# qinjr/SCoRe

Measured on AMD Instinct MI355X. Metric: train samples/sec @ batch=1024, higher is better.
Workload: dtype f32

## Files before the change

### score_amd/csrc/embed.hip

```cpp
#include <string.h>
#include "common.h"
#include "kernels.h"

__global__ void gather_rows_kernel(const float* __restrict__ table, int D4, const int32_t* __restrict__ idx,
                                   int64_t n_chunks, float* __restrict__ out) {
  int64_t i = (int64_t)blockIdx.x * blockDim.x + threadIdx.x;
  int64_t stride = (int64_t)gridDim.x * blockDim.x;
  for (; i < n_chunks; i += stride) {
    int64_t r = i / D4;
    int c = (int)(i - r * D4);
    int64_t row = idx[r];
    st4(out + i * 4, ld4(table + (row * D4 + c) * 4));
  }
}

extern "C" int score_gather_fwd(const float* table, int64_t n_rows, int32_t D, const int32_t* idx,
                                int64_t n_idx, float* out, void* stream) {
  if (!table || !idx || !out || n_rows <= 0 || n_idx < 0) return SCORE_E_BADARG;
  if (D <= 0 || (D & 3)) return SCORE_E_SHAPE;
  if (n_idx == 0) return 0;
  int64_t n_chunks = n_idx * (D / 4);
  int blocks = (int)(cdiv64(n_chunks, 256) < 4096 ? cdiv64(n_chunks, 256) : 4096);
  hipLaunchKernelGGL(gather_rows_kernel, dim3(blocks), dim3(256), 0, (hipStream_t)stream, table, D / 4, idx,
                     n_chunks, out);
// ... 138 lines not shown
#pragma unroll
  for (int k = 0; k < KMAX; ++k) {
    r[k] = 0.f;
    if (k < K) {
      r[k] = fmaxf(red[k] + c, 0.f);
      rmax = fmaxf(rmax, r[k]);
      rsum += r[k];
    }
  }
  float p[KMAX];
  float den = 0.f;
#pragma unroll
  for (int k = 0; k < KMAX; ++k) {
    p[k] = (k < K) ? expf(r[k] - rmax) : 0.f;
    den += p[k];
  }
  const float inv_den = 1.0f / den;
#pragma unroll
  for (int j = 0; j < SPL; ++j) {
    if (!ok[j]) continue;
    float4 o = make_float4(0.f, 0.f, 0.f, 0.f);
#pragma unroll
    for (int k = 0; k < KMAX; ++k)
      if (k < K) o = fma4(p[k] * inv_den, v1[j][k], o);
    st4(cc.out1 + (int64_t)u * cc.ld1 + (gl + j * GS) * 4, o);
    const float fk = (float)K;
    st4(cc.out2 + (int64_t)u * cc.ld2 + (gl + j * GS) * 4,
        make_float4(sum2[j].x / fk, sum2[j].y / fk, sum2[j].z / fk, sum2[j].w / fk));
  }
  if (unit_ok) {
    for (int i = gl; i < 2 * K; i += GS) {
      float val = rsum;
      float rv = 0.f;
#pragma unroll
      for (int k = 0; k < KMAX; ++k)
        if (i == k) rv = r[k];
      if (i < K) {
        val = (float)K * rv;
        cc.rsave[(int64_t)u * K + i] = rv;
      }
      cc.info[(int64_t)u * cc.ldi + i] = val;
    }
  }
}

__device__ __forceinline__ void atomic_add4(float* d, float4 v) {
  atomicAdd(d, v.x); atomicAdd(d + 1, v.y); atomicAdd(d + 2, v.z); atomicAdd(d + 3, v.w);
}

__device__ __forceinline__ void rows_in_flight(float4& row, const float4& last) {
  asm volatile("" : "+v"(row.x), "+v"(row.y), "+v"(row.z), "+v"(row.w) : "v"(last.w));
}

template <int KMAX, int SPL, bool ATOMIC>
__global__ __launch_bounds__(256, (KMAX <= 10 && SPL == 1) ? 4 : 1) void coattn_bwd_kernel_t(const CoattnArgs a) {
  extern __shared__ float lds[];
  const int ci = (int)blockIdx.x >= a.c[1].first_block ? 1 : 0;
  const CoattnCall& cc = a.c[ci];
  const int GS = cc.GS, nslots = cc.nslots, F = cc.F, K = a.K, D4 = a.D4, n_units = a.n_units;
  const int mode = a.mode;
  const bool all_rows = a.all_rows != 0;
  const int lane = threadIdx.x & 63;
  const int wib = threadIdx.x >> 6;
  const int upw = 64 / GS;
  const int gl = lane & (GS - 1);
  const int grp = lane / GS;
  const int Dx = nslots * 4;
  const int D = D4 * 4;
  const int my_blocks = (ci == 0 ? min(a.c[1].first_block, (int)gridDim.x) : (int)gridDim.x) - cc.first_block;
  const int waves_total = my_blocks * 4;
  const int blk = (int)blockIdx.x - cc.first_block;
  const int wave0 = blk * 4 + wib;
  const float* __restrict__ table = a.table;
  float* __restrict__ gtable = a.gtable;
  const float* __restrict__ W = cc.W;

  bool sok[SPL];
  int f[SPL], coff[SPL];
  float4 w1[SPL], w2[SPL], dw1[SPL], dw2[SPL];
#pragma unroll
  for (int j = 0; j < SPL; ++j) {
    int s = gl + j * GS;
    sok[j] = s < nslots;
    int sc = sok[j] ? s : 0;
    f[j] = sc / D4;
    coff[j] = (sc - f[j] * D4) * 4;
    w1[j] = w2[j] = dw1[j] = dw2[j] = make_float4(0.f, 0.f, 0.f, 0.f);
    if (mode == 0) {
      w1[j] = ld4(W + Dx + sc * 4);
      w2[j] = ld4(W + 2 * Dx + sc * 4);
    }
  }

  const int n_iter = (n_units + waves_total * upw - 1) / (waves_total * upw);
  for (int it = 0; it < n_iter; ++it) {
    const int unit = (it * waves_total + wave0) * upw + grp;
    const bool unit_ok = unit < n_units;
    const int u = unit_ok ? unit : 0;
    const int ub = u / a.T;
    const int64_t ui = (int64_t)ub * a.Tidx + (u - ub * a.T);
    const int32_t* __restrict__ i1 = cc.idx1 + ui * K * F;
    const int32_t* __restrict__ i2 = cc.idx2 + ui * K * F;
    float4 g1[SPL], g2[SPL];
    bool ok[SPL];
#pragma unroll
    for (int j = 0; j < SPL; ++j) {
      ok[j] = unit_ok && sok[j];
      g1[j] = g2[j] = make_float4(0.f, 0.f, 0.f, 0.f);
      if (ok[j]) {
        g1[j] = ld4(cc.g1 + (int64_t)u * cc.ld1 + (gl + j * GS) * 4);
        g2[j] = ld4(cc.g2 + (int64_t)u * cc.ld2 + (gl + j * GS) * 4);
      }
    }
    if (mode == 1) {
#pragma unroll
      for (int k = 0; k < KMAX; ++k) {
#pragma unroll
        for (int j = 0; j < SPL; ++j) {
          if (!ok[j] || k >= K) continue;
          if (!ATOMIC) continue;
          int64_t r1 = i1[k * F + f[j]], r2 = i2[k * F + f[j]];
          r1 = (uint64_t)r1 < a.n_rows ? r1 : 0;
          r2 = (uint64_t)r2 < a.n_rows ? r2 : 0;
          if (r1 != 0) atomic_add4(gtable + r1 * D + coff[j], g1[j]);
          if (r2 != 0) atomic_add4(gtable + r2 * D + coff[j], g2[j]);
        }
      }
      continue;
    }

    int32_t r1[SPL][KMAX], rb2[SPL][KMAX];
    float dp[KMAX];
#pragma unroll
    for (int k = 0; k < KMAX; ++k) {
      const int kc = k < K ? k : K - 1;
#pragma unroll
      for (int j = 0; j < SPL; ++j) {
        r1[j][k] = i1[kc * F + f[j]];
        rb2[j][k] = i2[kc * F + f[j]];
      }
    }
    __builtin_amdgcn_sched_barrier(0);
#pragma unroll
    for (int k = 0; k < KMAX; ++k) {
      dp[k] = 0.f;
#pragma unroll
      for (int j = 0; j < SPL; ++j) {
        r1[j][k] = (uint32_t)r1[j][k] < a.n_rows ? r1[j][k] : 0;
        rb2[j][k] = (uint32_t)rb2[j][k] < a.n_rows ? rb2[j][k] : 0;
      }
    }
#pragma unroll
    for (int j = 0; j < SPL; ++j) {
      float4 v1[KMAX];
#pragma unroll
      for (int k = 0; k < KMAX; ++k) v1[k] = ld4(table + (int64_t)r1[j][k] * D + coff[j]);
#pragma unroll
      for (int k = 0; k < KMAX; ++k) rows_in_flight(v1[k], v1[KMAX - 1]);
#pragma unroll
      for (int k = 0; k < KMAX; ++k) {
        const bool live = ok[j] && k < K;
        v1[k].x = live ? v1[k].x : 0.f; v1[k].y = live ? v1[k].y : 0.f;
        v1[k].z = live ? v1[k].z : 0.f; v1[k].w = live ? v1[k].w : 0.f;
        r1[j][k] = live ? r1[j][k] : 0;
        rb2[j][k] = live ? rb2[j][k] : 0;
        dp[k] += dot4(v1[k], g1[j]);
      }
    }
    float r[KMAX], p[KMAX], gik[KMAX];
    float rmax = 0.f, gsum = 0.f;
#pragma unroll
    for (int k = 0; k < KMAX; ++k) {
      const int kc = k < K ? k : K - 1;
      const float rv = cc.rsave[(int64_t)u * K + kc];
      const float g2v = cc.ginfo[(int64_t)u * cc.ldi + K + kc];
      gik[k] = cc.ginfo[(int64_t)u * cc.ldi + kc];
      r[k] = (k < K) ? rv : 0.f;
      rmax = fmaxf(rmax, r[k]);
      gsum += (k < K) ? g2v : 0.f;
    }
    float den = 0.f;
#pragma unroll
    for (int k = 0; k < KMAX; ++k) {
      p[k] = (k < K) ? expf(r[k] - rmax) : 0.f;
      den += p[k];
    }
    const float inv_den = 1.0f / den;
    float pdp = 0.f;
    group_sum_n<KMAX>(dp, GS);
#pragma unroll
    for (int k = 0; k < KMAX; ++k) {
      p[k] *= inv_den;
      dp[k] = (k < K) ? dp[k] : 0.f;
      pdp += p[k] * dp[k];
    }
    float dz[KMAX];
    float dzs = 0.f;
#pragma unroll
    for (int k = 0; k < KMAX; ++k) {
      dz[k] = 0.f;
      if (k < K) {
        float dr = (float)K * gik[k] + gsum + p[k] * (dp[k] - pdp);
        dz[k] = r[k] > 0.f ? dr : 0.f;
        dzs += dz[k];
      }
    }
    if (unit_ok && gl == 0) cc.dzsum[u] = dzs;
    if (!ATOMIC && unit_ok) {
      for (int i = gl; i < K; i += GS) {
        float pv = 0.f, dv = 0.f;
#pragma unroll
        for (int k = 0; k < KMAX; ++k)
          if (i == k) { pv = p[k]; dv = dz[k]; }
        cc.pcoef[(int64_t)u * K + i] = pv;
        cc.dzcoef[(int64_t)u * K + i] = dv;
      }
    }
    const float invK = 1.0f / (float)K;
    bool act[KMAX];
#pragma unroll
    for (int k = 0; k < KMAX; ++k) act[k] = all_rows || (k < K && r[k] > 0.f);
#pragma unroll
    for (int j = 0; j < SPL; ++j) {
      float4 xr[KMAX];
#pragma unroll
      for (int k = 0; k < KMAX; ++k) {
        const int32_t lr = act[k] ? r1[j][k] : 0;
        xr[k] = ld4(table + (int64_t)lr * D + coff[j]);
      }
#pragma unroll
      for (int k = 0; k < KMAX; ++k) {
        dw1[j] = fma4(dz[k], xr[k], dw1[j]);
        if (ATOMIC && r1[j][k] != 0) {
          float4 d1 = fma4(dz[k], w1[j],
                           make_float4(p[k] * g1[j].x, p[k] * g1[j].y, p[k] * g1[j].z, p[k] * g1[j].w));
          atomic_add4(gtable + (int64_t)r1[j][k] * D + coff[j], d1);
        }
      }
    }
#pragma unroll
    for (int j = 0; j < SPL; ++j) {
      const float4 g2k = make_float4(g2[j].x * invK, g2[j].y * invK, g2[j].z * invK, g2[j].w * invK);
      float4 y[KMAX];
#pragma unroll
      for (int k = 0; k < KMAX; ++k) {
        const int32_t lr = act[k] ? rb2[j][k] : 0;
        y[k] = ld4(table + (int64_t)lr * D + coff[j]);
      }
#pragma unroll
      for (int k = 0; k < KMAX; ++k) {
        dw2[j] = fma4(dz[k], y[k], dw2[j]);
        if (ATOMIC && rb2[j][k] != 0) atomic_add4(gtable + (int64_t)rb2[j][k] * D + coff[j], fma4(dz[k], w2[j], g2k));
      }
    }
  }
  if (mode == 1) return;
  float* mine = lds + ((wib * upw + grp) * 2) * Dx;
#pragma unroll
  for (int j = 0; j < SPL; ++j) {
    if (!sok[j]) continue;
    st4(mine + (gl + j * GS) * 4, dw1[j]);
    st4(mine + Dx + (gl + j * GS) * 4, dw2[j]);
  }
  __syncthreads();
  const int nsrc = 4 * upw;
  for (int e = threadIdx.x; e < 2 * Dx; e += blockDim.x) {
    float s = 0.f;
    for (int q = 0; q < nsrc; ++q) s += lds[q * 2 * Dx + e];
    cc.slab[(int64_t)blk * 2 * Dx + e] = s;
  }
}

#define COATTN_DISPATCH(KERNEL, EXTRA, SPLV, KV, ...)                                     \
  do {                                                                                    \
    if (SPLV == 1) {                                                                      \
      if (KV <= 4) { hipLaunchKernelGGL((KERNEL<4, 1 EXTRA>), __VA_ARGS__); }             \
      else if (KV <= 10) { hipLaunchKernelGGL((KERNEL<10, 1 EXTRA>), __VA_ARGS__); }      \
      else if (KV <= 20) { hipLaunchKernelGGL((KERNEL<20, 1 EXTRA>), __VA_ARGS__); }      \
      else { hipLaunchKernelGGL((KERNEL<32, 1 EXTRA>), __VA_ARGS__); }                    \
    } else if (SPLV == 2) {                                                               \
      if (KV <= 4) { hipLaunchKernelGGL((KERNEL<4, 2 EXTRA>), __VA_ARGS__); }             \
      else if (KV <= 10) { hipLaunchKernelGGL((KERNEL<10, 2 EXTRA>), __VA_ARGS__); }      \
      else if (KV <= 20) { hipLaunchKernelGGL((KERNEL<20, 2 EXTRA>), __VA_ARGS__); }      \
      else { hipLaunchKernelGGL((KERNEL<32, 2 EXTRA>), __VA_ARGS__); }                    \
    } else {                                                                              \
      if (KV <= 10) { hipLaunchKernelGGL((KERNEL<10, 4 EXTRA>), __VA_ARGS__); }           \
      else { hipLaunchKernelGGL((KERNEL<20, 4 EXTRA>), __VA_ARGS__); }                    \
    }                                                                                     \
  } while (0)
#define COMMA_TRUE , true
#define COMMA_FALSE , false

static int coattn_check(const void* table, int64_t n_rows, int D, int F, int K, int B, int T) {
  if (!table || n_rows <= 0 || B <= 0 || T <= 0) return SCORE_E_BADARG;
  if (D <= 0 || (D & 3) || D > 256 || F <= 0 || K <= 0 || K > 32) return SCORE_E_SHAPE;
  if (F * (D / 4) > 256) return SCORE_E_SHAPE;
  if (F * (D / 4) > 128 && K > 20) return SCORE_E_SHAPE;
  return 0;
}

int score_coattn_fwd_multi(CoattnArgs& a, int ncalls, int D, int B, hipStream_t s) {
  int spl = 1, total = 0;
  a.D4 = D / 4;
  a.n_units = B * a.T;
  if (a.Tidx <= 0) a.Tidx = a.T;
  if (a.n_rows == 0) a.n_rows = 0x80000000u;
  for (int c = 0; c < 2; ++c) {
    if (c >= ncalls) { a.c[c] = a.c[0]; a.c[c].first_block = 0x7fffffff; continue; }
    int SPLc;
    coattn_geom(D, a.c[c].F, &a.c[c].GS, &SPLc, &a.c[c].nslots);
    if (SPLc > spl) spl = SPLc;
    a.c[c].first_block = total;
    total += (int)cdiv64(cdiv64(a.n_units, 64 / a.c[c].GS), 4);
  }
  if (spl == 3) spl = 4;
  COATTN_DISPATCH(coattn_fwd_kernel, , spl, a.K, dim3(total), dim3(256), 0, s, a);
  SCORE_CHECK_LAUNCH();
  return 0;
}

int score_coattn_bwd_multi(CoattnArgs& a, int ncalls, int D, int B, float* const dW[2], float* scratch,
                           int64_t scratch_floats, int atomic_scatter, ColsumJobs* cq, hipStream_t s) {
  int spl = 1, total = 0, nblk[2] = {0, 0};
  size_t lds_bytes = 0;
  int64_t used = 0;
  a.D4 = D / 4;
  a.n_units = B * a.T;
  if (a.Tidx <= 0) a.Tidx = a.T;
  if (a.n_rows == 0) a.n_rows = 0x80000000u;
  for (int c = 0; c < 2; ++c) {
    if (c >= ncalls) { a.c[c] = a.c[0]; a.c[c].first_block = 0x7fffffff; continue; }
    int SPLc;
    coattn_geom(D, a.c[c].F, &a.c[c].GS, &SPLc, &a.c[c].nslots);
    if (SPLc > spl) spl = SPLc;
    int upw = 64 / a.c[c].GS, Dx = a.c[c].nslots * 4;
    int blocks = (int)cdiv64(cdiv64(a.n_units, upw), 4);
    if (blocks > 512) blocks = 512;
    nblk[c] = blocks;
    a.c[c].first_block = total;
    total += blocks;
    a.c[c].slab = scratch + used;
    used += (int64_t)blocks * 2 * Dx;
    size_t l = (size_t)4 * upw * 2 * Dx * sizeof(float);
    if (l > lds_bytes) lds_bytes = l;
  }
  if (a.mode == 0 && used > scratch_floats) return SCORE_E_WORKSPACE;
  if (spl == 3) spl = 4;
  if (atomic_scatter) COATTN_DISPATCH(coattn_bwd_kernel_t, COMMA_TRUE, spl, a.K, dim3(total), dim3(256), lds_bytes, s, a);
  else COATTN_DISPATCH(coattn_bwd_kernel_t, COMMA_FALSE, spl, a.K, dim3(total), dim3(256), lds_bytes, s, a);
  SCORE_CHECK_LAUNCH();
  if (a.mode == 0) {
    for (int c = 0; c < ncalls; ++c) {
      int Dx = a.c[c].nslots * 4;
      if (cq) SCORE_TRY(colsum_queue_add(cq, a.c[c].slab, nblk[c], 2 * Dx, 2 * Dx, dW[c] + Dx, 1));
      else SCORE_TRY(score_launch_colsum(a.c[c].slab, nblk[c], 2 * Dx, 2 * Dx, dW[c] + Dx, 1, scratch + used,
                                         scratch_floats - used, s));
    }
  }
  return 0;
}

extern "C" int score_coattn_fwd(const float* table, int64_t n_rows, int32_t D, int32_t F, int32_t K,
                                int32_t B, int32_t T, const int32_t* idx1, const int32_t* idx2,
                                const float* tgt, const float* W, const float* bias, float* out1,
                                int32_t ld1, float* out2, int32_t ld2, float* info, int32_t ldi,
                                float* rsave, int32_t mode, void* stream) {
  SCORE_TRY(coattn_check(table, n_rows, D, F, K, B, T));
  if (!idx1 || !idx2 || !out1 || !out2) return SCORE_E_BADARG;
  if (mode == 0 && (!tgt || !W || !bias || !info || !rsave)) return SCORE_E_BADARG;
  if ((ld1 & 3) || (ld2 & 3)) return SCORE_E_SHAPE;
  CoattnArgs a;
  memset(&a, 0, sizeof(a));
  a.table = table; a.K = K; a.T = T; a.mode = mode; a.n_rows = (uint32_t)(n_rows < 0x80000000ll ? n_rows : 0x80000000ll);
  CoattnCall& c = a.c[0];
  c.idx1 = idx1; c.idx2 = idx2; c.tgt = tgt; c.ldt = F * D; c.W = W; c.bias = bias;
  c.out1 = out1; c.ld1 = ld1; c.out2 = out2; c.ld2 = ld2; c.info = info; c.ldi = ldi; c.rsave = rsave; c.F = F;
  return score_coattn_fwd_multi(a, 1, D, B, (hipStream_t)stream);
}

extern "C" int score_coattn_bwd(const float* table, float* grad_table, int64_t n_rows, int32_t D, int32_t F,
                                int32_t K, int32_t B, int32_t T, const int32_t* idx1, const int32_t* idx2,
                                const float* W, const float* rsave, const float* g1, int32_t ld1,
                                const float* g2, int32_t ld2, const float* ginfo, int32_t ldi, float* dzsum,
                                float* dW, float* scratch, int64_t scratch_floats, int32_t mode, void* stream) {
  SCORE_TRY(coattn_check(table, n_rows, D, F, K, B, T));
  if (!grad_table || !idx1 || !idx2 || !g1 || !g2) return SCORE_E_BADARG;
  if (mode == 0 && (!W || !rsave || !ginfo || !dzsum || !dW || !scratch)) return SCORE_E_BADARG;
  if ((ld1 & 3) || (ld2 & 3)) return SCORE_E_SHAPE;
  CoattnArgs a;
  memset(&a, 0, sizeof(a));
  a.table = table; a.gtable = grad_table; a.K = K; a.T = T; a.mode = mode;
  a.n_rows = (uint32_t)(n_rows < 0x80000000ll ? n_rows : 0x80000000ll);
  CoattnCall& c = a.c[0];
  c.idx1 = idx1; c.idx2 = idx2; c.W = W; c.rsave = const_cast<float*>(rsave); c.g1 = g1; c.ld1 = ld1; c.g2 = g2; c.ld2 = ld2;
  c.ginfo = ginfo; c.ldi = ldi; c.dzsum = dzsum; c.F = F;
  float* dWs[2] = {dW, nullptr};
  return score_coattn_bwd_multi(a, 1, D, B, dWs, scratch, scratch_floats, 1, nullptr, (hipStream_t)stream);
}

__global__ void target_fwd_kernel(const float* __restrict__ table, int D4, int Fu, int Fi, int B,
                                  const int32_t* __restrict__ tu, const int32_t* __restrict__ ti,
                                  float* __restrict__ query, int ldq, float* __restrict__ head, int ldh,
// ... 126 lines not shown
```

### score_amd/csrc/engine.hip

```cpp
#include <string.h>
#include <stdlib.h>
#include <stdio.h>
#include <math.h>
#include <mutex>
#include <new>
#include "common.h"
#include "kernels.h"
#include "persample.h"

namespace {

const int FC1 = 200, FC2 = 80, AT1 = 80, AT2 = 40;
const int CASER_L = SCORE_CASER_L, CASER_HPAD = SCORE_CASER_HPAD;
const int MAX_ENTRIES = 48;

enum Family { FAM_SLICE, FAM_GCMC, FAM_G4R, FAM_CASER, FAM_DELF, FAM_DEEMS, FAM_SVDPP, FAM_SASREC };

struct Dims {
  int64_t N;
  int D, H, T, K, Fu, Fi, mt;
  int Du, Di, I, Dq, NI, Dk, Dhead, nstate;
  int Is[2];
  bool coattn, attn;
  Family family;
// ... 468 lines not shown
  HIPTRY(hipEventRecord((hipEvent_t)event, (hipStream_t)stream));
  return 0;
}
extern "C" int score_stream_wait_event(void* stream, void* event) {
  if (!event) return SCORE_E_BADARG;
  HIPTRY(hipStreamWaitEvent((hipStream_t)stream, (hipEvent_t)event, 0));
  return 0;
}
extern "C" int score_event_query(void* event) {
  if (!event) return SCORE_E_BADARG;
  const hipError_t e = hipEventQuery((hipEvent_t)event);
  return e == hipSuccess ? 0 : e == hipErrorNotReady ? 1 : (int)e;
}
extern "C" int score_event_synchronize(void* event) {
  if (!event) return SCORE_E_BADARG;
  HIPTRY(hipEventSynchronize((hipEvent_t)event));
  return 0;
}
static int side_stream_create(SideStream* sd) {
  int dev = 0;
  if (hipGetDevice(&dev) != hipSuccess) return SCORE_E_BADARG;
  hipStream_t st; hipEvent_t a, b, c;
  hipError_t e = hipStreamCreateWithFlags(&st, hipStreamNonBlocking);
  if (e != hipSuccess) return (int)e;
  if ((e = hipEventCreateWithFlags(&a, SCORE_DEVICE_EVENT_FLAGS)) != hipSuccess) { hipStreamDestroy(st); return (int)e; }
  if ((e = hipEventCreateWithFlags(&b, SCORE_DEVICE_EVENT_FLAGS)) != hipSuccess) { hipEventDestroy(a); hipStreamDestroy(st); return (int)e; }
  if ((e = hipEventCreateWithFlags(&c, SCORE_DEVICE_EVENT_FLAGS)) != hipSuccess) { hipEventDestroy(a); hipEventDestroy(b); hipStreamDestroy(st); return (int)e; }
  sd->st = st; sd->fork = a; sd->join = b; sd->wx = c; sd->device = dev; sd->fwd_on = nullptr;
  return 0;
}
static void side_stream_release(SideStream* sd) {
  if (!sd->st) return;
  hipStreamSynchronize(sd->st);
  hipEventDestroy(sd->fork); hipEventDestroy(sd->join); hipEventDestroy(sd->wx);
  hipStreamDestroy(sd->st);
  sd->st = nullptr;
}
#define SCORE_MAX_DEVICES 16
static SideStream g_default_ctx[SCORE_MAX_DEVICES];
static std::mutex g_default_mu;
static int side_stream(const score_state_t* st, SideStream** out) {
  if (st && st->context) { *out = reinterpret_cast<SideStream*>(st->context); return 0; }
  int dev = 0;
  if (hipGetDevice(&dev) != hipSuccess || dev < 0 || dev >= SCORE_MAX_DEVICES) return SCORE_E_BADARG;
  std::lock_guard<std::mutex> lock(g_default_mu);
  SideStream& sd = g_default_ctx[dev];
  if (!sd.st) SCORE_TRY(side_stream_create(&sd));
  *out = &sd;
  return 0;
}
enum {
  DF_GRU_STEPWISE = 1, DF_HEAD_FUSED_ANY_B = 2, DF_GRU_F32_REC = 4, DF_NO_PANEL = 8, DF_PANEL_DX = 16, DF_SORT_LIB = 32,
  DF_HEAD_UNFUSED = 64, DF_ATTN_UNFUSED = 128, DF_SORT_OWN = 256, DF_NO_PS = 512, DF_PS_FWD_ONLY = 1024, DF_PS_BWD_ONLY = 2048,
  DF_ONE_STREAM = 4096, DF_G4R_COMPOSED = 8192, DF_PRODUCTS_LATE = 16384, DF_COATTN_ALL_ROWS = 32768
};
struct Flags {
  bool gru_stepwise, head_fused_any_b, gru_f32_rec, no_panel, panel_dx, sort_lib, head_unfused, attn_unfused, sort_own, no_ps,
      ps_fwd_only, ps_bwd_only, one_stream, g4r_composed, products_late, coattn_all_rows;
};
static inline Flags flags_of(const score_state_t* st) {
  auto on = [st](int bit) { return (st->debug_flags & bit) != 0; };
  Flags o;
  o.gru_stepwise = on(DF_GRU_STEPWISE); o.head_fused_any_b = on(DF_HEAD_FUSED_ANY_B); o.gru_f32_rec = on(DF_GRU_F32_REC);
  o.no_panel = on(DF_NO_PANEL); o.panel_dx = on(DF_PANEL_DX); o.sort_lib = on(DF_SORT_LIB); o.sort_own = on(DF_SORT_OWN);
  o.head_unfused = on(DF_HEAD_UNFUSED); o.attn_unfused = on(DF_ATTN_UNFUSED); o.no_ps = on(DF_NO_PS);
  o.ps_fwd_only = on(DF_PS_FWD_ONLY); o.ps_bwd_only = on(DF_PS_BWD_ONLY); o.one_stream = on(DF_ONE_STREAM);
  o.g4r_composed = on(DF_G4R_COMPOSED); o.products_late = on(DF_PRODUCTS_LATE); o.coattn_all_rows = on(DF_COATTN_ALL_ROWS);
  return o;
}
static int side_stream(const score_state_t* st, hipStream_t s, SideStream** out) {
  SideStream* real = nullptr;
  SCORE_TRY(side_stream(st, &real));
  if (!st || !flags_of(st).one_stream) { *out = real; return 0; }
  static thread_local SideStream inl;
  const hipStream_t was = inl.fwd_on;
  inl = *real; inl.st = s; inl.fwd_on = was;
  *out = &inl;
  return 0;
}
static inline int fork_side(SideStream* side, hipStream_t s) {
  HIPTRY(hipEventRecord(side->fork, s));
  HIPTRY(hipStreamWaitEvent(side->st, side->fork, 0));
  return 0;
}

#define G(call) SCORE_TRY(call)
static inline int gemm_mode_call(int x3, int tr, int M, int N, int K, const float* A, int lda, const float* B,
                                 int ldb, float* C, int ldc, const float* bias, int flags, float keep,
                                 const uint8_t* mask, uint64_t seed, float* scratch, int64_t scratch_floats,
                                 void* s) {
  return score_gemm(tr, M, N, K, A, lda, B, ldb, C, ldc, bias, flags | x3, keep, mask, seed, scratch, scratch_floats,
                    s);
}
#define EV(i) \
  do { if (stage_events && stage_events[i]) HIPTRY(hipEventRecord((hipEvent_t)stage_events[i], s)); } while (0)

static inline uint32_t clamp_rows(int64_t n) { return (uint32_t)(n < 0x80000000ll ? n : 0x80000000ll); }
static inline int global_batch(const score_state_t* st, int B) { return st->global_batch > 0 ? st->global_batch : B; }

struct Pass {
  Dims d; Params P; WS w; Flags fl;
  const score_state_t* st; const score_batch_t* bt;
  int B, T, BT, H;
  int x3, Bg;
  uint32_t n_rows;
  int64_t weff_stride;
  float rs;
  float* ws; const float* W; float* scratch;
  hipStream_t s;
};
static int pass_fill(Pass* c, const score_state_t* st, const score_batch_t* bt, void* stream) {
  const Dims& d = c->d;
  build_layout(d, nullptr, 0, &c->P);
  c->st = st; c->bt = bt; c->fl = flags_of(st);
  c->B = bt->B; c->T = active_T(d, bt); c->H = d.H; c->BT = c->B * c->T;
  build_ws(d, c->B, &c->w);
  if (c->w.total * 4 > st->workspace_bytes) return SCORE_E_WORKSPACE;
  c->x3 = st->gemm_mode == 1 ? GF_X3 : 0; c->Bg = global_batch(st, c->B); c->n_rows = clamp_rows(st->n_table_rows);
  c->weff_stride = weff_copy_stride(d); c->rs = (float)(1.0 / sqrt(1.0 + 1e-3));
  c->ws = st->workspace; c->W = st->w; c->scratch = c->ws + c->w.scratch;
// ... 1292 lines not shown
    HIPTRY(hipMemsetAsync(ws + w.dxside[sd], 0, (int64_t)BT * d.I * sizeof(float), s));
    const int Dx = d.Is[sd];
    float* dz = ws + w.gcmc_dz[sd];
    float* da = ws + w.gcmc_da[sd];
    G(gemm_mode_call(x3, 1, BT, Dx, 3 * H, ws + w.dxproj[sd], 3 * H, wxcat(c, sd), 3 * H, dz, Dx, nullptr, GF_RELUGRAD, 1.f,
                     reinterpret_cast<const uint8_t*>(ws + w.gcmc_z[sd]), 0, c.scratch, SF, s));
    G(gemm_queue_add(&gq, Dx, Dx, BT, ws + w.gcmc_a[sd], Dx, dz, Dx, gw + P.gm_c[sd], Dx));
    G(gemm_mode_call(x3, 1, BT, Dx, Dx, dz, Dx, W + P.gm_c[sd], Dx, da, Dx, nullptr, GF_RELUGRAD, 1.f,
                     reinterpret_cast<const uint8_t*>(ws + w.gcmc_a[sd]), 0, c.scratch, SF, s));
    G(gemm_queue_add(&gq, Dx, Dx, BT, ws + w.xside[sd], d.I, da, Dx, gw + P.gm_a[sd], Dx));
    G(gemm_mode_call(x3, 1, BT, Dx, Dx, da, Dx, W + P.gm_a[sd], Dx, ws + w.dxside[sd], d.I, nullptr, 0, 1.f, nullptr, 0,
                     c.scratch, SF, s));
  }
  return 0;
}

int bwd_dx_g4r(const Pass& c, BwdState* b) {
  const Dims& d = c.d; const WS& w = c.w; float* ws = c.ws; const int H = c.H, BT = c.BT; hipStream_t s = c.s;
  G(queue_gru_side(c, &b->q, b->gw, 0, b->gru_bias_rows));
  HIPTRY(hipMemsetAsync(ws + w.dxside[0], 0, (int64_t)BT * d.I * sizeof(float), s));
  G(gemm_mode_call(c.x3, 1, BT, d.Di, 3 * H, ws + w.dxproj[0], 3 * H, wxcat(c, 0), 3 * H, ws + w.dxside[0], d.I, nullptr, 0, 1.f,
                   nullptr, 0, c.scratch, w.scratch_floats, s));
  G(queue_gru_side(c, &b->q, b->gw, 1, b->gru_bias_rows));
  HIPTRY(hipMemsetAsync(ws + w.dxside[1], 0, (int64_t)BT * d.I * sizeof(float), s));
  return 0;
}

int bwd_close(const Pass& c, BwdState* b) {
  const Dims& d = c.d; const Params& P = c.P; const WS& w = c.w; const score_state_t* st = c.st; const score_batch_t* bt = c.bt;
  float* ws = c.ws; const float* W = c.W; float* gw = b->gw; float* grad_table = b->grad_table;
  const int B = c.B, x3 = c.x3; hipStream_t s = c.s;
  void* const* stage_events = b->stage_events;
  SideStream* side = b->side;
  GemmQueue& gq = b->q.gq;
  ColsumJobs& cq = b->q.cq;
  const int64_t half = slab_half(w);
  ReduceGroup rg; rg.n = rg.blocks = 0;
  const bool products_early = st->scatter_mode != 2 && !c.fl.products_late && gq.n > 0;
  const bool fin_side = st->grads_done_event != nullptr;
  const bool fin_early = products_early && fin_side;
  if (products_early) {
    G(fork_side(side, s));
    G(gemm_queue_flush(&gq, x3 != 0, ws + w.dwslab + half, w.dwslab_floats - half, side->st, &rg));
    HIPTRY(hipEventRecord(side->join, side->st));
  }
  EV(3);
  const bool atomic = st->scatter_mode == 1;
  {
    CoattnArgs ca;
    CoattnCols k;
    coattn_args(c, &ca, &k);
    ca.gtable = grad_table;
    ca.all_rows = c.fl.coattn_all_rows ? 1 : 0;
    for (int i = 0; i < 2; ++i) {
      CoattnCall& cc = ca.c[i];
      cc.g1 = ws + w.dxside[0] + k.col1[i]; cc.g2 = ws + w.dxside[1] + k.col2[i]; cc.ginfo = ws + w.dinfo + k.info_col[i];
      cc.dzsum = ws + w.dzsum[i]; cc.pcoef = ws + w.pcoef[i]; cc.dzcoef = ws + w.dzcoef[i];
    }
    float* dWs[2] = {d.coattn ? gw + P.ca_w[0] : nullptr, d.coattn ? gw + P.ca_w[1] : nullptr};
    if (atomic || d.coattn)
      G(score_coattn_bwd_multi(ca, 2, d.D, B, dWs, ws + w.ca_slab, w.ca_slab_floats, atomic ? 1 : 0, &cq, s));
  }
  if (d.attn && st->scatter_mode != 2) HIPTRY(hipStreamWaitEvent(s, side->wx, 0));
  if (!atomic && st->plan_done_event) HIPTRY(hipStreamWaitEvent(s, (hipEvent_t)st->plan_done_event, 0));
  if (!d.reads_targets) {
    if (!atomic) HIPTRY(hipMemsetAsync(ws + w.dtgt, 0, (int64_t)B * d.Dq * sizeof(float), s));
  } else
  G(score_launch_target_bwd(grad_table, d.D, d.Fu, d.Fi, B, c.T, bt->target_user, bt->target_item,
                            d.attn ? ws + w.dquery : nullptr, d.Dq, ws + w.dhead, d.Dhead, d.off_ti, d.off_tu,
                            ws + w.query, d.coattn ? W + P.ca_w[0] : nullptr, d.coattn ? W + P.ca_w[1] : nullptr,
                            ws + w.dzsum[0], ws + w.dzsum[1], ws + w.S, d.coattn ? gw + P.ca_w[0] : nullptr,
                            d.coattn ? gw + P.ca_b[0] : nullptr, d.coattn ? gw + P.ca_w[1] : nullptr,
                            d.coattn ? gw + P.ca_b[1] : nullptr, atomic ? nullptr : ws + w.dtgt, c.scratch, w.scratch_floats, &cq, &gq,
                            s, st->n_table_rows));
  float* cs_part2 = ws + w.cs_part + w.cs_part_floats / 2;
  const int64_t cs_part2_floats = w.cs_part_floats - w.cs_part_floats / 2;
  if (fin_early) {
    G(fork_side(side, s));
    G(score_launch_finish(&rg, &cq, cs_part2, cs_part2_floats, side->st, 0));
    HIPTRY(hipEventRecord((hipEvent_t)st->grads_done_event, side->st));
    HIPTRY(hipEventRecord(side->join, side->st));
  }
  if (!atomic) G(row_scatter(c, (st->plan_workspace && st->scatter_mode == 0) ? st->plan_workspace : ws, grad_table));
  EV(4);
  HIPTRY(hipStreamWaitEvent(s, side->join, 0));
  if (!products_early) G(gemm_queue_flush(&gq, x3 != 0, ws + w.dwslab + half, w.dwslab_floats - half, s, &rg));
  EV(5);
  if (fin_early) return 0;
  if (fin_side) G(fork_side(side, s));
  hipStream_t fs = fin_side ? side->st : s;
  G(score_launch_finish(&rg, &cq, cs_part2, cs_part2_floats, fs, 0));
  if (fin_side) HIPTRY(hipEventRecord((hipEvent_t)st->grads_done_event, fs));
  return 0;
}

int bwd_slice(const Pass& c, BwdState* b) {
  hipStream_t s = c.s;
  void* const* stage_events = b->stage_events;
  G(bwd_open(c, b));
  G(bwd_fc_head(c, b));
  EV(1);
  if (c.d.attn) G(bwd_attention(c, b));
  else G(bwd_final_states(c, b, true));
  EV(2);
  G(bwd_side_products(c, b));
  G(bwd_grus_two_sided(c, b));
// ... 176 lines not shown
```

### score_amd/csrc/kernels.h

```cpp
#pragma once
#include "common.h"

#define GEMM_GROUP_MAX 16
struct GemmProb {
  const float* A; const float* B; float* C; float* slab;
  const float* bias;
  int M, N, K, lda, ldb, ldc, k_chunk, gx, gy, nblocks;
};
struct GemmGroup { int n; int total_blocks; GemmProb p[GEMM_GROUP_MAX]; };
enum { GF_BIAS = 1, GF_RELU = 2, GF_ACC = 4, GF_DROP = 8, GF_X3 = 16, GF_X3F = 32, GF_RELUGRAD = 64 };
__device__ __forceinline__ int64_t bias_index(int flags, int row, int col, int N) {
  const int g = flags >> 16;
  return g ? (int64_t)(row / g) * N + col : col;
}
__device__ __forceinline__ float gemm_epilogue(float v, int row, int col, int N, const float* bias, int flags,
                                               float keep, const uint8_t* mask, uint64_t seed) {
  if (flags & GF_BIAS) v += bias[bias_index(flags, row, col, N)];
  if (flags & GF_RELU) v = fmaxf(v, 0.f);
  if (flags & GF_DROP) {
    uint64_t e = (uint64_t)row * (uint64_t)N + (uint64_t)col;
    bool on = mask ? (mask[e] != 0) : (hash_uniform(seed, e) < keep);
    v = on ? v / keep : 0.f;
  }
  if (flags & GF_RELUGRAD) {
    const float y = reinterpret_cast<const float*>(mask)[(int64_t)row * N + col];
    v = y > 0.f ? v / keep : 0.f;
  }
  return v;
}
int score_launch_gemm_bf16x3(int trans, int wm, const GemmGroup& g, const float* bias, int flags, float keep,
                             const uint8_t* mask, uint64_t seed, hipStream_t s);
struct GemmQueueJob { const float* A; const float* B; float* C; int M, N, K, lda, ldb, ldc; };
struct GemmQueue { int n; GemmQueueJob j[2 * GEMM_GROUP_MAX]; };
int gemm_queue_add(GemmQueue* q, int M, int N, int K, const float* A, int lda, const float* B, int ldb, float* C,
                   int ldc);
struct ReduceJob { const float* slab; float* C; int ns, M, N, ldc, first_block, pad; };
struct ReduceGroup { int n; int blocks; ReduceJob j[2 * GEMM_GROUP_MAX]; };
struct ColsumJobs;
int gemm_queue_flush(GemmQueue* q, int x3, float* slab, int64_t slab_floats, hipStream_t s, ReduceGroup* defer = nullptr,
                     const ColsumJobs* with_colsums = nullptr, float* cs_part = nullptr, int64_t cs_part_floats = 0,
                     int* colsums_done = nullptr);
#define COLSUM_MAX_JOBS 24
#define COLSUM_MAX_PARTS 128
struct ColsumJob { const float* X; float* out; const float* scale; int M, N, ld, acc, cols, rpb, nparts; int64_t part_off; };
struct ColsumJobs { ColsumJob job[COLSUM_MAX_JOBS]; int n; int64_t part_used; };
int colsum_queue_add(ColsumJobs* q, const float* X, int M, int N, int ld, float* out, int acc, const float* scale = nullptr);
int colsum_queue_flush(ColsumJobs* q, float* part, int64_t part_floats, hipStream_t s);
struct W1Fold { int Dk, NA; const float* dweff; const float* dwq; float* gW1; const float* slab_e; const float* slab_q; int ns_e, ns_q; };
int score_launch_finish(const ReduceGroup* rg, ColsumJobs* q, float* part, int64_t part_floats, hipStream_t s, int stage1_done = 0,
                        const W1Fold* w1 = nullptr);
int score_launch_colsum(const float* X, int M, int N, int ld, float* out, int accumulate,
                        float* scratch, int64_t scratch_floats, hipStream_t s);
struct CoattnCall {
  const int32_t* idx1; const int32_t* idx2;
  const float* tgt; int ldt;
  const int32_t* tidx;
  const float* W; const float* bias;
  float* out1; int ld1; float* out2; int ld2;
  float* info; int ldi; float* rsave;
  const float* g1; const float* g2; const float* ginfo;
  float* dzsum; float* slab;
  float* pcoef; float* dzcoef;
  int F, GS, nslots, first_block;
  int bit1, bit2;
};
struct CoattnArgs {
  CoattnCall c[2];
  const float* table; float* gtable;
  int D4, K, T, n_units, mode;
  int Tidx;
  uint32_t n_rows; int32_t* id_status;
  int all_rows;
};
int score_coattn_fwd_multi(CoattnArgs& a, int ncalls, int D, int B, hipStream_t s);
int score_coattn_bwd_multi(CoattnArgs& a, int ncalls, int D, int B, float* const dW[2], float* scratch,
                           int64_t scratch_floats, int atomic_scatter, ColsumJobs* cq, hipStream_t s);
int score_launch_target_fwd(const float* table, int D, int Fu, int Fi, int B, const int32_t* tu,
                            const int32_t* ti, float* query, int ldq, float* head, int ldh,
                            int off_ti, int off_tu, hipStream_t s, int64_t n_rows = 0, int32_t* id_status = nullptr);
int score_launch_target_bwd(float* grad_table, int D, int Fu, int Fi, int B, int T, const int32_t* tu,
                            const int32_t* ti, const float* dquery, int ldq, const float* dhead, int ldh,
                            int off_ti, int off_tu, const float* query, const float* W1, const float* W2,
                            const float* dzsum1, const float* dzsum2, float* S ,
                            float* dW1, float* dB1, float* dW2, float* dB2, float* dtgt_out, float* scratch,
                            int64_t scratch_floats, ColsumJobs* cq, struct GemmQueue* gq, hipStream_t s,
                            int64_t n_rows = 0);
int score_launch_attn_build_inp(int B, int T, int H, int NI, const float* q, const float* ur, const float* ir,
                                const float* info, float* inp, hipStream_t s);
int score_launch_attn_pool_fwd(int B, int T, int H, int NA, const float* a2, const float* w5, const float* b5,
                               const int32_t* length, const float* ur, const float* ir, float* score, float* head,
                               int ldh, int off_u, int off_i, hipStream_t s);
int score_launch_attn_tail_fwd(int B, int T, int H, int N1, int N2, const float* a1, const float* W4, const float* b4,
                               const float* w5, const float* b5, const int32_t* length, const float* ur, const float* ir,
                               float* a2, float* score, float* head, int ldh, int off_u, int off_i, hipStream_t s);
int score_launch_attn_pool_bwd(int B, int T, int H, int NA, const float* a2, const float* w5,
                               const int32_t* length, const float* ur, const float* ir, const float* score,
                               const float* dhead, int ldh, int off_u, int off_i, float* ds, float* da2,
                               hipStream_t s, int N1 = 0, const float* W4 = nullptr, const float* a1 = nullptr,
                               float* da1 = nullptr);
int score_launch_attn_inp_bwd(int B, int T, int H, int NI, const float* dinp, const float* q, const float* ur,
                              const float* ir, const float* info, const float* score, const float* dhead, int ldh,
                              int off_u, int off_i, const float* dqd, float* dur, float* dir, float* dinfo, float* dq,
                              hipStream_t s);
int score_launch_attn_inp_bwd_fused(int B, int T, int H, int NI, int N1, const float* da1, const float* Weff, const float* q,
                                    const float* ur, const float* ir, const float* info, const float* score,
                                    const float* dhead, int ldh, int off_u, int off_i, float* dur, float* dir, float* dinfo,
                                    float* dq, hipStream_t s, int N2 = 0, const float* a2 = nullptr, const float* a1 = nullptr,
                                    const float* w5 = nullptr, const float* W4 = nullptr, const int32_t* length = nullptr,
                                    float* ds = nullptr, float* da2 = nullptr, float* da1_out = nullptr);
bool score_attn_inp_bwd_fused_fits(int B, int T, int H, int NI, int N1, int N2, int ldh, int off_u, int off_i, bool pool);
#define SCORE_WEFF_COPIES 8
int score_launch_attn_dzsum(int B, int T, int NA, const float* dz, float* dzsum, hipStream_t s);
int score_launch_attn_w1_grad(int Dk, int NA, const float* dweff, const float* dwq, float* gW1, hipStream_t s);
int score_launch_bn_fwd(int B, int Dh, const float* x, const float* gamma, const float* beta, float rs, float* y,
                        hipStream_t s);
int score_launch_bn_bwd(int B, int Dh, const float* x, const float* gamma, float rs, const float* dy, float* dx,
                        float* dgamma, float* dbeta, float* tmp, float* scratch, int64_t scratch_floats,
                        ColsumJobs* cq, hipStream_t s);
int score_launch_weight_prep(const float* gk0, const float* ck0, const float* gb0, const float* cb0, const float* gk1,
                             const float* ck1, const float* gb1, const float* cb1, int I0, int I1, int Imax, int H, float* cat,
                             int Dk, int NA, const float* W1, float* weff, float* wq, int copies, int64_t copy_stride,
                             const float* wreg, int64_t n_reg, float* part, hipStream_t s);
int score_launch_head_out(int B, int NF, const float* f2, const float* w3, const float* b3, const int32_t* label,
                          float* logit, float* y, float* lossb, float* dlogit, float* loss, float lambda,
                          const float* part, int Bglobal, hipStream_t s, const int32_t* id_status = nullptr);
// ... 195 lines not shown
```

Measured before the change: 946,700.

## Load co-attention backward per-unit metadata cooperatively and distribute via ds_bpermute

The co-attention backward kernel gets a new template path where each lane group loads a unit's row indices and saved scalars (rsave, ginfo) once, spread across lanes in a few registers. Each lane then fetches the values it needs through ds_bpermute instead of issuing many redundant scalar global loads. An optional debug flag also prefetches the next unit's metadata during the current iteration. This targets latency and redundant traffic from index and scalar loads, at the cost of cross-lane shuffles, extra template instantiations and more register pressure.

```diff
diff --git a/score_amd/csrc/embed.hip b/score_amd/csrc/embed.hip
--- a/score_amd/csrc/embed.hip
+++ b/score_amd/csrc/embed.hip
@@ -214,19 +214,108 @@
   asm volatile("" : "+v"(row.x), "+v"(row.y), "+v"(row.z), "+v"(row.w) : "v"(last.w));
 }
 
-template <int KMAX, int SPL, bool ATOMIC>
+
+static inline int coattn_ksh(int GS, int F) {
+  if (F > GS) return -1;
+  int sh = 0;
+  while ((2 << sh) * F <= GS) ++sh;
+  return sh;
+}
+static inline int coattn_meta_regs(int GS, int F, int K) {
+  const int ksh = coattn_ksh(GS, F);
+  if (ksh < 0) return 0;
+  const int ids = (K + (1 << ksh) - 1) >> ksh, sc = (3 * K + GS - 1) / GS;
+  return ids > sc ? ids : sc;
+}
+
+template <typename T> struct MetaList { T r0, r1, r2, r3; };
+struct UnitMeta { MetaList<int32_t> a, b; MetaList<float> s; };
+template <int I, typename T> __device__ __forceinline__ T& meta_at(MetaList<T>& l) {
+  if constexpr (I == 0) return l.r0;
+  else if constexpr (I == 1) return l.r1;
+  else if constexpr (I == 2) return l.r2;
+  else return l.r3;
+}
+template <int NM, typename T>
+__device__ __forceinline__ T meta_reg(const MetaList<T>& l, int reg) {
+  static_assert(NM >= 1 && NM <= 4, "a list is at most four registers");
+  T v = l.r0;
+  if constexpr (NM > 1) { const T x = l.r1; v = reg == 1 ? x : v; }
+  if constexpr (NM > 2) { const T x = l.r2; v = reg == 2 ? x : v; }
+  if constexpr (NM > 3) { const T x = l.r3; v = reg == 3 ? x : v; }
+  return v;
+}
+
+template <int I>
+__device__ __forceinline__ void unit_meta_load1(UnitMeta& m, const int32_t* __restrict__ i1, const int32_t* __restrict__ i2,
+                                                const float* __restrict__ rs, const float* __restrict__ gi, int K, int KF,
+                                                int GS, int per, int gc, int gl) {
+  const int e = I * per + gc, es = I * GS + gl;
+  const int ei = e < KF ? e : KF - 1;
+  const int esc = es < 3 * K ? es : 3 * K - 1;
+  meta_at<I>(m.a) = i1[ei];
+  meta_at<I>(m.b) = i2[ei];
+  meta_at<I>(m.s) = *(esc < K ? rs + esc : gi + (esc - K));
+}
+template <int I>
+__device__ __forceinline__ void unit_meta_clamp1(UnitMeta& m, uint32_t n_rows) {
+  const int32_t x = meta_at<I>(m.a), y = meta_at<I>(m.b);
+  meta_at<I>(m.a) = (uint32_t)x < n_rows ? x : 0;
+  meta_at<I>(m.b) = (uint32_t)y < n_rows ? y : 0;
+}
+template <int NM>
+__device__ __forceinline__ void unit_meta_load(UnitMeta& m, const CoattnArgs& a, const CoattnCall& cc, int u, int gl) {
+  const int K = a.K, KF = a.K * cc.F, GS = cc.GS, per = cc.F << cc.ksh;
+  const int ub = u / a.T;
+  const int64_t ui = (int64_t)ub * a.Tidx + (u - ub * a.T);
+  const int32_t* __restrict__ i1 = cc.idx1 + ui * KF;
+  const int32_t* __restrict__ i2 = cc.idx2 + ui * KF;
+  const float* __restrict__ rs = cc.rsave + (int64_t)u * K;
+  const float* __restrict__ gi = cc.ginfo + (int64_t)u * cc.ldi;
+  const int gc = gl < per ? gl : per - 1;
+  unit_meta_load1<0>(m, i1, i2, rs, gi, K, KF, GS, per, gc, gl);
+  if constexpr (NM > 1) unit_meta_load1<1>(m, i1, i2, rs, gi, K, KF, GS, per, gc, gl);
+  if constexpr (NM > 2) unit_meta_load1<2>(m, i1, i2, rs, gi, K, KF, GS, per, gc, gl);
+  if constexpr (NM > 3) unit_meta_load1<3>(m, i1, i2, rs, gi, K, KF, GS, per, gc, gl);
+  unit_meta_clamp1<0>(m, a.n_rows);
+  if constexpr (NM > 1) unit_meta_clamp1<1>(m, a.n_rows);
+  if constexpr (NM > 2) unit_meta_clamp1<2>(m, a.n_rows);
+  if constexpr (NM > 3) unit_meta_clamp1<3>(m, a.n_rows);
+}
+
+#define META_RECOMPUTE(vgpr, sgpr0, sgpr1) asm volatile("" : "+v"(vgpr), "+s"(sgpr0), "+s"(sgpr1))
+
+template <int KMAX, int NM>
+__device__ __forceinline__ void unit_ids(int32_t (&out)[KMAX], const MetaList<int32_t>& l, int K, int F, int ksh, int fj, int gbase) {
+  META_RECOMPUTE(gbase, K, F);
+#pragma unroll
+  for (int k = 0; k < KMAX; ++k) {
+    const int kc = k < K ? k : K - 1;
+    const int reg = kc >> ksh;
+    out[k] = __builtin_amdgcn_ds_bpermute((gbase + (kc - (reg << ksh)) * F + fj) << 2, meta_reg<NM>(l, reg));
+  }
+}
+
+template <int NM>
+__device__ __forceinline__ float unit_scalar(const MetaList<float>& l, int e, int gbase, int GS, int gsh) {
+  return __int_as_float(__builtin_amdgcn_ds_bpermute((gbase + (e & (GS - 1))) << 2, __float_as_int(meta_reg<NM>(l, e >> gsh))));
+}
+
+template <int KMAX, int SPL, bool ATOMIC, int NM>
 __global__ __launch_bounds__(256, (KMAX <= 10 && SPL == 1) ? 4 : 1) void coattn_bwd_kernel_t(const CoattnArgs a) {
   extern __shared__ float lds[];
   const int ci = (int)blockIdx.x >= a.c[1].first_block ? 1 : 0;
   const CoattnCall& cc = a.c[ci];
   const int GS = cc.GS, nslots = cc.nslots, F = cc.F, K = a.K, D4 = a.D4, n_units = a.n_units;
   const int mode = a.mode;
-  const bool all_rows = a.all_rows != 0;
+  const bool all_rows = a.all_rows != 0, ahead = a.meta_ahead != 0;
   const int lane = threadIdx.x & 63;
   const int wib = threadIdx.x >> 6;
   const int upw = 64 / GS;
   const int gl = lane & (GS - 1);
   const int grp = lane / GS;
+  const int gbase = lane - gl;
+  const int gsh = __builtin_ctz(GS), ksh = cc.ksh;
   const int Dx = nslots * 4;
   const int D = D4 * 4;
   const int my_blocks = (ci == 0 ? min(a.c[1].first_block, (int)gridDim.x) : (int)gridDim.x) - cc.first_block;
@@ -255,6 +344,13 @@
   }
 
   const int n_iter = (n_units + waves_total * upw - 1) / (waves_total * upw);
+  UnitMeta cur;
+  if constexpr (NM > 0) {
+    if (ahead) {
+      const int unit = wave0 * upw + grp;
+      unit_meta_load<NM>(cur, a, cc, unit < n_units ? unit : 0, gl);
+    }
+  }
   for (int it = 0; it < n_iter; ++it) {
     const int unit = (it * waves_total + wave0) * upw + grp;
     const bool unit_ok = unit < n_units;
@@ -266,12 +362,15 @@
     float4 g1[SPL], g2[SPL];
     bool ok[SPL];
 #pragma unroll
-    for (int j = 0; j < SPL; ++j) {
-      ok[j] = unit_ok && sok[j];
-      g1[j] = g2[j] = make_float4(0.f, 0.f, 0.f, 0.f);
-      if (ok[j]) {
-        g1[j] = ld4(cc.g1 + (int64_t)u * cc.ld1 + (gl + j * GS) * 4);
-        g2[j] = ld4(cc.g2 + (int64_t)u * cc.ld2 + (gl + j * GS) * 4);
+    for (int j = 0; j < SPL; ++j) ok[j] = unit_ok && sok[j];
+    if (NM == 0 || mode == 1) {
+#pragma unroll
+      for (int j = 0; j < SPL; ++j) {
+        g1[j] = g2[j] = make_float4(0.f, 0.f, 0.f, 0.f);
+        if (ok[j]) {
+          g1[j] = ld4(cc.g1 + (int64_t)u * cc.ld1 + (gl + j * GS) * 4);
+          g2[j] = ld4(cc.g2 + (int64_t)u * cc.ld2 + (gl + j * GS) * 4);
+        }
       }
     }
     if (mode == 1) {
@@ -293,50 +392,91 @@
 
     int32_t r1[SPL][KMAX], rb2[SPL][KMAX];
     float dp[KMAX];
-#pragma unroll
-    for (int k = 0; k < KMAX; ++k) {
-      const int kc = k < K ? k : K - 1;
+    UnitMeta nxt;
+    if constexpr (NM > 0) {
+      if (!ahead) unit_meta_load<NM>(cur, a, cc, u, gl);
 #pragma unroll
       for (int j = 0; j < SPL; ++j) {
-        r1[j][k] = i1[kc * F + f[j]];
-        rb2[j][k] = i2[kc * F + f[j]];
-      }
-    }
-    __builtin_amdgcn_sched_barrier(0);
-#pragma unroll
-    for (int k = 0; k < KMAX; ++k) {
-      dp[k] = 0.f;
-#pragma unroll
-      for (int j = 0; j < SPL; ++j) {
-        r1[j][k] = (uint32_t)r1[j][k] < a.n_rows ? r1[j][k] : 0;
-        rb2[j][k] = (uint32_t)rb2[j][k] < a.n_rows ? rb2[j][k] : 0;
-      }
-    }
+        const int sc = sok[j] ? gl + j * GS : 0;
+        g1[j] = ld4(cc.g1 + (int64_t)u * cc.ld1 + sc * 4);
+        g2[j] = ld4(cc.g2 + (int64_t)u * cc.ld2 + sc * 4);
+      }
+    } else {
+#pragma unroll
+      for (int k = 0; k < KMAX; ++k) {
+        const int kc = k < K ? k : K - 1;
+#pragma unroll
+        for (int j = 0; j < SPL; ++j) {
+          r1[j][k] = i1[kc * F + f[j]];
+          rb2[j][k] = i2[kc * F + f[j]];
+        }
+      }
+      __builtin_amdgcn_sched_barrier(0);
+#pragma unroll
+      for (int k = 0; k < KMAX; ++k) {
+#pragma unroll
+        for (int j = 0; j < SPL; ++j) {
+          r1[j][k] = (uint32_t)r1[j][k] < a.n_rows ? r1[j][k] : 0;
+          rb2[j][k] = (uint32_t)rb2[j][k] < a.n_rows ? rb2[j][k] : 0;
+        }
+      }
+    }
+#pragma unroll
+    for (int k = 0; k < KMAX; ++k) dp[k] = 0.f;
 #pragma unroll
     for (int j = 0; j < SPL; ++j) {
+      if constexpr (NM > 0) unit_ids<KMAX, NM>(r1[j], cur.a, K, F, ksh, f[j], gbase);
       float4 v1[KMAX];
 #pragma unroll
       for (int k = 0; k < KMAX; ++k) v1[k] = ld4(table + (int64_t)r1[j][k] * D + coff[j]);
+      if constexpr (NM > 0) {
+        if (j == 0) {
+          if (ahead) {
+            const int64_t unit_n = ((int64_t)(it + 1) * waves_total + wave0) * upw + grp;
+            unit_meta_load<NM>(nxt, a, cc, unit_n < n_units ? (int)unit_n : 0, gl);
+          }
+          __builtin_amdgcn_sched_barrier(0);
+        }
+      }
 #pragma unroll
       for (int k = 0; k < KMAX; ++k) rows_in_flight(v1[k], v1[KMAX - 1]);
+      if constexpr (NM > 0) {
+        g1[j].x = ok[j] ? g1[j].x : 0.f; g1[j].y = ok[j] ? g1[j].y : 0.f;
+        g1[j].z = ok[j] ? g1[j].z : 0.f; g1[j].w = ok[j] ? g1[j].w : 0.f;
+        g2[j].x = ok[j] ? g2[j].x : 0.f; g2[j].y = ok[j] ? g2[j].y : 0.f;
+        g2[j].z = ok[j] ? g2[j].z : 0.f; g2[j].w = ok[j] ? g2[j].w : 0.f;
+        asm volatile("" : "+v"(g2[j].x), "+v"(g2[j].y), "+v"(g2[j].z), "+v"(g2[j].w));
+      }
 #pragma unroll
       for (int k = 0; k < KMAX; ++k) {
         const bool live = ok[j] && k < K;
         v1[k].x = live ? v1[k].x : 0.f; v1[k].y = live ? v1[k].y : 0.f;
         v1[k].z = live ? v1[k].z : 0.f; v1[k].w = live ? v1[k].w : 0.f;
-        r1[j][k] = live ? r1[j][k] : 0;
-        rb2[j][k] = live ? rb2[j][k] : 0;
+        if constexpr (NM == 0) {
+          r1[j][k] = live ? r1[j][k] : 0;
+          rb2[j][k] = live ? rb2[j][k] : 0;
+        }
         dp[k] += dot4(v1[k], g1[j]);
       }
     }
     float r[KMAX], p[KMAX], gik[KMAX];
     float rmax = 0.f, gsum = 0.f;
+    int gb_s = gbase, K_s = K, GS_s = GS;
+    if constexpr (NM > 0) META_RECOMPUTE(gb_s, K_s, GS_s);
 #pragma unroll
     for (int k = 0; k < KMAX; ++k) {
       const int kc = k < K ? k : K - 1;
-      const float rv = cc.rsave[(int64_t)u * K + kc];
-      const float g2v = cc.ginfo[(int64_t)u * cc.ldi + K + kc];
-      gik[k] = cc.ginfo[(int64_t)u * cc.ldi + kc];
+      float rv, g2v;
+      if constexpr (NM > 0) {
+        const int kcs = k < K_s ? k : K_s - 1;
+        rv = unit_scalar<NM>(cur.s, kcs, gb_s, GS_s, gsh);
+        gik[k] = unit_scalar<NM>(cur.s, K_s + kcs, gb_s, GS_s, gsh);
+        g2v = unit_scalar<NM>(cur.s, 2 * K_s + kcs, gb_s, GS_s, gsh);
+      } else {
+        rv = cc.rsave[(int64_t)u * K + kc];
+        g2v = cc.ginfo[(int64_t)u * cc.ldi + K + kc];
+        gik[k] = cc.ginfo[(int64_t)u * cc.ldi + kc];
+      }
       r[k] = (k < K) ? rv : 0.f;
       rmax = fmaxf(rmax, r[k]);
       gsum += (k < K) ? g2v : 0.f;
@@ -385,10 +525,19 @@
 #pragma unroll
     for (int j = 0; j < SPL; ++j) {
       float4 xr[KMAX];
+      if constexpr (NM > 0) {
+        unit_ids<KMAX, NM>(r1[j], cur.a, K, F, ksh, f[j], gbase);
+#pragma unroll
+        for (int k = 0; k < KMAX; ++k) r1[j][k] = (ok[j] && k < K) ? r1[j][k] : 0;
+      }
 #pragma unroll
       for (int k = 0; k < KMAX; ++k) {
         const int32_t lr = act[k] ? r1[j][k] : 0;
         xr[k] = ld4(table + (int64_t)lr * D + coff[j]);
+      }
+      if constexpr (NM > 0) {
+#pragma unroll
+        for (int k = 0; k < KMAX; ++k) rows_in_flight(xr[k], xr[KMAX - 1]);
       }
 #pragma unroll
       for (int k = 0; k < KMAX; ++k) {
@@ -404,16 +553,28 @@
     for (int j = 0; j < SPL; ++j) {
       const float4 g2k = make_float4(g2[j].x * invK, g2[j].y * invK, g2[j].z * invK, g2[j].w * invK);
       float4 y[KMAX];
+      if constexpr (NM > 0) {
+        unit_ids<KMAX, NM>(rb2[j], cur.b, K, F, ksh, f[j], gbase);
+#pragma unroll
+        for (int k = 0; k < KMAX; ++k) rb2[j][k] = (ok[j] && k < K) ? rb2[j][k] : 0;
+      }
 #pragma unroll
       for (int k = 0; k < KMAX; ++k) {
         const int32_t lr = act[k] ? rb2[j][k] : 0;
         y[k] = ld4(table + (int64_t)lr * D + coff[j]);
       }
+      if constexpr (NM > 0) {
+#pragma unroll
+        for (int k = 0; k < KMAX; ++k) rows_in_flight(y[k], y[KMAX - 1]);
+      }
 #pragma unroll
       for (int k = 0; k < KMAX; ++k) {
         dw2[j] = fma4(dz[k], y[k], dw2[j]);
         if (ATOMIC && rb2[j][k] != 0) atomic_add4(gtable + (int64_t)rb2[j][k] * D + coff[j], fma4(dz[k], w2[j], g2k));
       }
+    }
+    if constexpr (NM > 0) {
+      if (ahead) cur = nxt;
     }
   }
   if (mode == 1) return;
@@ -450,8 +611,29 @@
       else { hipLaunchKernelGGL((KERNEL<20, 4 EXTRA>), __VA_ARGS__); }                    \
     }                                                                                     \
   } while (0)
-#define COMMA_TRUE , true
-#define COMMA_FALSE , false
+#define COMMA_TRUE0 , true, 0
+#define COMMA_FALSE0 , false, 0
+template <int KMAX, int SPL, bool ATOMIC, int NM>
+static void coattn_bwd_launch(int total, size_t lds_bytes, hipStream_t s, const CoattnArgs& a) {
+  hipLaunchKernelGGL((coattn_bwd_kernel_t<KMAX, SPL, ATOMIC, NM>), dim3(total), dim3(256), lds_bytes, s, a);
+}
+template <int SPL, bool ATOMIC>
+static bool coattn_bwd_ahead(int need, int total, size_t lds_bytes, hipStream_t s, const CoattnArgs& a) {
+  const int K = a.K;
+  if (need < 1 || need > 4) return false;
+  if (K <= 4) {
+    if (need > 2) return false;
+    if (need == 1) coattn_bwd_launch<4, SPL, ATOMIC, 1>(total, lds_bytes, s, a);
+    else coattn_bwd_launch<4, SPL, ATOMIC, 2>(total, lds_bytes, s, a);
+  } else if (K <= 10) {
+    if (need == 1) coattn_bwd_launch<10, SPL, ATOMIC, 1>(total, lds_bytes, s, a);
+    else if (need == 2) coattn_bwd_launch<10, SPL, ATOMIC, 2>(total, lds_bytes, s, a);
+    else coattn_bwd_launch<10, SPL, ATOMIC, 4>(total, lds_bytes, s, a);
+  } else {
+    return false;
+  }
+  return true;
+}
 
 static int coattn_check(const void* table, int64_t n_rows, int D, int F, int K, int B, int T) {
   if (!table || n_rows <= 0 || B <= 0 || T <= 0) return SCORE_E_BADARG;
@@ -508,8 +690,20 @@
   }
   if (a.mode == 0 && used > scratch_floats) return SCORE_E_WORKSPACE;
   if (spl == 3) spl = 4;
-  if (atomic_scatter) COATTN_DISPATCH(coattn_bwd_kernel_t, COMMA_TRUE, spl, a.K, dim3(total), dim3(256), lds_bytes, s, a);
-  else COATTN_DISPATCH(coattn_bwd_kernel_t, COMMA_FALSE, spl, a.K, dim3(total), dim3(256), lds_bytes, s, a);
+  int need = (a.mode == 0 && spl <= 2) ? 1 : 0;
+  for (int c = 0; c < ncalls && need > 0; ++c) {
+    const int n = coattn_meta_regs(a.c[c].GS, a.c[c].F, a.K);
+    need = n == 0 ? 0 : n > need ? n : need;
+  }
+  for (int c = 0; c < 2; ++c) a.c[c].ksh = need > 0 ? coattn_ksh(a.c[c].GS, a.c[c].F) : 0;
+  bool ahead;
+  if (spl == 1) ahead = atomic_scatter ? coattn_bwd_ahead<1, true>(need, total, lds_bytes, s, a) : coattn_bwd_ahead<1, false>(need, total, lds_bytes, s, a);
+  else if (spl == 2) ahead = atomic_scatter ? coattn_bwd_ahead<2, true>(need, total, lds_bytes, s, a) : coattn_bwd_ahead<2, false>(need, total, lds_bytes, s, a);
+  else ahead = false;
+  if (!ahead) {
+    if (atomic_scatter) COATTN_DISPATCH(coattn_bwd_kernel_t, COMMA_TRUE0, spl, a.K, dim3(total), dim3(256), lds_bytes, s, a);
+    else COATTN_DISPATCH(coattn_bwd_kernel_t, COMMA_FALSE0, spl, a.K, dim3(total), dim3(256), lds_bytes, s, a);
+  }
   SCORE_CHECK_LAUNCH();
   if (a.mode == 0) {
     for (int c = 0; c < ncalls; ++c) {
diff --git a/score_amd/csrc/engine.hip b/score_amd/csrc/engine.hip
--- a/score_amd/csrc/engine.hip
+++ b/score_amd/csrc/engine.hip
@@ -544,11 +544,12 @@
 enum {
   DF_GRU_STEPWISE = 1, DF_HEAD_FUSED_ANY_B = 2, DF_GRU_F32_REC = 4, DF_NO_PANEL = 8, DF_PANEL_DX = 16, DF_SORT_LIB = 32,
   DF_HEAD_UNFUSED = 64, DF_ATTN_UNFUSED = 128, DF_SORT_OWN = 256, DF_NO_PS = 512, DF_PS_FWD_ONLY = 1024, DF_PS_BWD_ONLY = 2048,
-  DF_ONE_STREAM = 4096, DF_G4R_COMPOSED = 8192, DF_PRODUCTS_LATE = 16384, DF_COATTN_ALL_ROWS = 32768
+  DF_ONE_STREAM = 4096, DF_G4R_COMPOSED = 8192, DF_PRODUCTS_LATE = 16384, DF_COATTN_ALL_ROWS = 32768,
+  DF_COATTN_META_AHEAD = 65536
 };
 struct Flags {
   bool gru_stepwise, head_fused_any_b, gru_f32_rec, no_panel, panel_dx, sort_lib, head_unfused, attn_unfused, sort_own, no_ps,
-      ps_fwd_only, ps_bwd_only, one_stream, g4r_composed, products_late, coattn_all_rows;
+      ps_fwd_only, ps_bwd_only, one_stream, g4r_composed, products_late, coattn_all_rows, coattn_meta_ahead;
 };
 static inline Flags flags_of(const score_state_t* st) {
   auto on = [st](int bit) { return (st->debug_flags & bit) != 0; };
@@ -558,6 +559,7 @@
   o.head_unfused = on(DF_HEAD_UNFUSED); o.attn_unfused = on(DF_ATTN_UNFUSED); o.no_ps = on(DF_NO_PS);
   o.ps_fwd_only = on(DF_PS_FWD_ONLY); o.ps_bwd_only = on(DF_PS_BWD_ONLY); o.one_stream = on(DF_ONE_STREAM);
   o.g4r_composed = on(DF_G4R_COMPOSED); o.products_late = on(DF_PRODUCTS_LATE); o.coattn_all_rows = on(DF_COATTN_ALL_ROWS);
+  o.coattn_meta_ahead = on(DF_COATTN_META_AHEAD);
   return o;
 }
 static int side_stream(const score_state_t* st, hipStream_t s, SideStream** out) {
@@ -1956,6 +1958,7 @@
     coattn_args(c, &ca, &k);
     ca.gtable = grad_table;
     ca.all_rows = c.fl.coattn_all_rows ? 1 : 0;
+    ca.meta_ahead = c.fl.coattn_meta_ahead ? 1 : 0;
     for (int i = 0; i < 2; ++i) {
       CoattnCall& cc = ca.c[i];
       cc.g1 = ws + w.dxside[0] + k.col1[i]; cc.g2 = ws + w.dxside[1] + k.col2[i]; cc.ginfo = ws + w.dinfo + k.info_col[i];
diff --git a/score_amd/csrc/kernels.h b/score_amd/csrc/kernels.h
--- a/score_amd/csrc/kernels.h
+++ b/score_amd/csrc/kernels.h
@@ -62,6 +62,7 @@
   float* dzsum; float* slab;
   float* pcoef; float* dzcoef;
   int F, GS, nslots, first_block;
+  int ksh;
   int bit1, bit2;
 };
 struct CoattnArgs {
@@ -71,6 +72,7 @@
   int Tidx;
   uint32_t n_rows; int32_t* id_status;
   int all_rows;
+  int meta_ahead;
 };
 int score_coattn_fwd_multi(CoattnArgs& a, int ncalls, int D, int B, hipStream_t s);
 int score_coattn_bwd_multi(CoattnArgs& a, int ncalls, int D, int B, float* const dW[2], float* scratch,
```

Result: faster. 959,600 (median of 6 runs) (+1.4%).
